# nka77/DAHiTra

Hardware: NVIDIA B200
Metric: image-pairs/sec (higher is better)
Workload: dtype x3 error-compensated f16 products (f16 main + scaled-remainder corrections; decoder: 3xTF32), fp32 accumulate

## Files before the change

dahitra_b200/csrc/stem_tc.cu:

```cuda
#include "tc_common.cuh"

using namespace dhtc;

namespace {
constexpr int SK_TH = 8, SK_TW = 16;
constexpr int SK_HR = 2 * SK_TH + 5;
constexpr int SK_HCP = 40;
constexpr int SK_PLANE = SK_HR * SK_HCP;
constexpr int SK_KSTEPS = 6;
constexpr int SK_GROUPS = 21;
constexpr uint32_t SK_A_BYTES = 128 * 128;
constexpr uint32_t SK_B_BYTES = SK_KSTEPS * 64 * 128;
constexpr uint32_t SK_HALO_BYTES = 3 * SK_PLANE * 4;
constexpr uint32_t SK_HALO_STRIDE = 10112;
constexpr uint32_t SK_IDESC = umma_idesc_tf32(128, 64);
constexpr int SK_THREADS = 14 * 32;

template <bool X3> struct SkCfg {
  static constexpr uint32_t NA = X3 ? 4 : 2;
  static constexpr uint32_t NB = X3 ? 2 : 1;
  static constexpr uint32_t OFF_B = NA * SK_A_BYTES;
  static constexpr uint32_t OFF_H = OFF_B + NB * SK_B_BYTES;
  static constexpr uint32_t OFF_E = OFF_H + 2 * SK_HALO_STRIDE;
  static constexpr uint32_t SMEM = OFF_E + 4 * 4096 + 1024;
};

__device__ __forceinline__ float sk_tf32(float v) { return tf32_round(v); }

struct SkTile { int n, oy0, ox0; };
__device__ __forceinline__ SkTile sk_tile(int t, int tilesX, int tilesY) {
  SkTile r;
  r.ox0 = (t % tilesX) * SK_TW; t /= tilesX;
  r.oy0 = (t % tilesY) * SK_TH;
  r.n = t / tilesY;
  return r;
}

__device__ __forceinline__ void sk_halo_producer(const CUtensorMap* tmX, uint32_t halo_addr, uint64_t* halo_full, uint64_t* halo_free,
                                                 int tilesX, int tilesY, int ntiles, const CUtensorMap* tmX2 = nullptr, int nfirst = 1 << 30) {
  int it = 0;
  for (int tile = blockIdx.x; tile < ntiles; tile += gridDim.x, ++it) {
    const int hb = it & 1;
    if (it >= 2) mbar_wait(smem_u32(&halo_free[hb]), (uint32_t)(((it >> 1) - 1) & 1));
    const SkTile tl = sk_tile(tile, tilesX, tilesY);
    const uint32_t bar = smem_u32(&halo_full[hb]);
    mbar_expect_tx(bar, SK_HALO_BYTES);
    const bool second = tl.n >= nfirst;
    tma_load_4d(halo_addr + (uint32_t)hb * SK_HALO_STRIDE, second ? tmX2 : tmX, bar, 2 * tl.ox0 - 4, 2 * tl.oy0 - 3, 0, second ? tl.n - nfirst : tl.n);
  }
}

__device__ __forceinline__ void sk_store_slice(const float (&v)[32], float* stage, int lane, int q, int j, const SkTile& t,
                                               int OH, int OW, const float* __restrict__ bias, float* __restrict__ out,
                                               long long split_plane = 0) {
  const int c4 = lane & 3, r4 = lane >> 2;
#pragma unroll
  for (int k4 = 0; k4 < 8; ++k4)
    *reinterpret_cast<float4*>(stage + lane * 32 + ((k4 ^ (lane & 7)) << 2)) = make_float4(v[k4 * 4], v[k4 * 4 + 1], v[k4 * 4 + 2], v[k4 * 4 + 3]);
  __syncwarp();
  const float4 b0 = ldg4(bias + j * 32 + c4 * 8), b1 = ldg4(bias + j * 32 + c4 * 8 + 4);
#pragma unroll
  for (int g = 0; g < 4; ++g) {
    const int r = g * 8 + r4, mm = q * 32 + r;
    const int oy = t.oy0 + mm / SK_TW, ox = t.ox0 + mm % SK_TW;
    const float4 o0 = *reinterpret_cast<const float4*>(stage + r * 32 + (((2 * c4) ^ (r & 7)) << 2));
    const float4 o1 = *reinterpret_cast<const float4*>(stage + r * 32 + (((2 * c4 + 1) ^ (r & 7)) << 2));
    if (oy < OH && ox < OW) {
      const float4 r0 = make_float4(fmaxf(o0.x + b0.x, 0.f), fmaxf(o0.y + b0.y, 0.f), fmaxf(o0.z + b0.z, 0.f), fmaxf(o0.w + b0.w, 0.f));
      const float4 r1 = make_float4(fmaxf(o1.x + b1.x, 0.f), fmaxf(o1.y + b1.y, 0.f), fmaxf(o1.z + b1.z, 0.f), fmaxf(o1.w + b1.w, 0.f));
      const size_t off = ((size_t)(t.n * OH + oy) * OW + ox) * 64 + j * 32 + c4 * 8;
      if (split_plane < 0) {
        uint4 hi;
        hi.x = pack_f16x2_sat(r0.x, r0.y); hi.y = pack_f16x2_sat(r0.z, r0.w); hi.z = pack_f16x2_sat(r1.x, r1.y); hi.w = pack_f16x2_sat(r1.z, r1.w);
        *reinterpret_cast<uint4*>(reinterpret_cast<uint16_t*>(out) + off) = hi;
      } else if (split_plane) {
        uint4 hi, lo;
        hi.x = pack_f16x2_sat(r0.x, r0.y); hi.y = pack_f16x2_sat(r0.z, r0.w); hi.z = pack_f16x2_sat(r1.x, r1.y); hi.w = pack_f16x2_sat(r1.z, r1.w);
        lo.x = pack_f16x2_sat((r0.x - f16_lo(hi.x)) * 2048.f, (r0.y - f16_hi(hi.x)) * 2048.f);
        lo.y = pack_f16x2_sat((r0.z - f16_lo(hi.y)) * 2048.f, (r0.w - f16_hi(hi.y)) * 2048.f);
        lo.z = pack_f16x2_sat((r1.x - f16_lo(hi.z)) * 2048.f, (r1.y - f16_hi(hi.z)) * 2048.f);
        lo.w = pack_f16x2_sat((r1.z - f16_lo(hi.w)) * 2048.f, (r1.w - f16_hi(hi.w)) * 2048.f);
        uint16_t* o16 = reinterpret_cast<uint16_t*>(out);
        *reinterpret_cast<uint4*>(o16 + off) = hi;
        *reinterpret_cast<uint4*>(o16 + off + (size_t)split_plane) = lo;
      } else {
        st4(out + off, r0); st4(out + off + 4, r1);
      }
    }
  }
  __syncwarp();
}

template <bool X3>
__global__ void __launch_bounds__(SK_THREADS, 1)
stem_tc_kernel(const __grid_constant__ CUtensorMap tmX, int OH, int OW, int tilesX, int tilesY, int ntiles,
               const float* __restrict__ wtc, const float* __restrict__ bias, float* __restrict__ out) {
  using Cfg = SkCfg<X3>;
  extern __shared__ uint8_t sk_raw[];
  __shared__ __align__(8) uint64_t w_bar, a_full[2], a_free[2], acc_full[2], acc_empty[2], halo_full[2], halo_free[2];
  __shared__ uint32_t tmem_slot;
  const int tid = threadIdx.x, warp = tid >> 5;
  const uint32_t base = (smem_u32(sk_raw) + 1023u) & ~1023u;
  uint8_t* bp = sk_raw + (base - smem_u32(sk_raw));
  constexpr uint32_t A_LO = 2 * SK_A_BYTES;
  const uint32_t b_addr = base + Cfg::OFF_B;

  if (tid == 0) {
    mbar_init(smem_u32(&w_bar), 1);
    for (int i = 0; i < 2; ++i) {
      mbar_init(smem_u32(&a_full[i]), 128);
      mbar_init(smem_u32(&a_free[i]), 1);
      mbar_init(smem_u32(&acc_full[i]), 1);
      mbar_init(smem_u32(&acc_empty[i]), 128);
      mbar_init(smem_u32(&halo_full[i]), 1);
      mbar_init(smem_u32(&halo_free[i]), 256);
    }
    mbar_fence_init();
  }
  if (warp == 0) tmem_alloc(smem_u32(&tmem_slot), 128);
  tc_fence_before();
  __syncthreads();
  tc_fence_after();
  const uint32_t tmem_base = tmem_slot;

  if (warp < 8) {
    const int wg = warp >> 2, t = tid & 127;
    const int py = t / SK_TW, px = t % SK_TW;
    const int pbase = (2 * py) * SK_HCP + 2 * px;
    const int swz = t & 7;
    int it = 0, use = 0;
    for (int tile = blockIdx.x; tile < ntiles; tile += gridDim.x, ++it) {
      const int hb = it & 1;
      mbar_wait(smem_u32(&halo_full[hb]), (uint32_t)((it >> 1) & 1));
      const float* halo = reinterpret_cast<const float*>(bp + Cfg::OFF_H + (size_t)hb * SK_HALO_STRIDE) + pbase;
      float* at = reinterpret_cast<float*>(bp + (size_t)wg * SK_A_BYTES) + t * 32;
#pragma unroll 1
      for (int kt = wg; kt < SK_KSTEPS; kt += 2, ++use) {
        if (use >= 1) mbar_wait(smem_u32(&a_free[wg]), (uint32_t)((use - 1) & 1));
#pragma unroll
        for (int j = 0; j < 4; ++j) {
          const int g = kt * 4 + j;
          float v[8];
          if (g < SK_GROUPS) {
            const float2* src = reinterpret_cast<const float2*>(halo + (g / 7) * SK_PLANE + (g % 7) * SK_HCP);
#pragma unroll
            for (int q = 0; q < 4; ++q) { const float2 f = src[q]; v[2 * q] = f.x; v[2 * q + 1] = f.y; }
          } else {
#pragma unroll
            for (int q = 0; q < 8; ++q) v[q] = 0.f;
          }
#pragma unroll
          for (int c = 0; c < 2; ++c) {
            const int o = ((2 * j + c) ^ swz) << 2;
            const float h0 = sk_tf32(v[c * 4]), h1 = sk_tf32(v[c * 4 + 1]), h2 = sk_tf32(v[c * 4 + 2]), h3 = sk_tf32(v[c * 4 + 3]);
            *reinterpret_cast<float4*>(at + o) = make_float4(h0, h1, h2, h3);
            if (X3) *reinterpret_cast<float4*>(at + A_LO / 4 + o) = make_float4(sk_tf32(v[c * 4] - h0), sk_tf32(v[c * 4 + 1] - h1),
                                                                              sk_tf32(v[c * 4 + 2] - h2), sk_tf32(v[c * 4 + 3] - h3));
          }
        }
        fence_async_smem();
        mbar_arrive_local(smem_u32(&a_full[wg]));
      }
      mbar_arrive_local(smem_u32(&halo_free[hb]));
    }
  } else if (warp < 12) {
    const int q = warp & 3, lane = tid & 31;
    float* stage = reinterpret_cast<float*>(bp + Cfg::OFF_E + (size_t)q * 4096);
    int it = 0;
    for (int tile = blockIdx.x; tile < ntiles; tile += gridDim.x, ++it) {
      const SkTile t = sk_tile(tile, tilesX, tilesY);
      const int ab = it & 1;
      mbar_wait(smem_u32(&acc_full[ab]), (uint32_t)((it >> 1) & 1));
      tc_fence_after();
      const uint32_t tm = tmem_base + ((uint32_t)(q * 32) << 16) + (uint32_t)ab * 64;
#pragma unroll 1
      for (int j = 0; j < 2; ++j) {
        uint32_t u[32];
        float v[32];
        tmem_ld32(tm + (uint32_t)(j * 32), u);
        if (j == 1) {
          tc_fence_before();
          mbar_arrive_local(smem_u32(&acc_empty[ab]));
        }
#pragma unroll
        for (int i = 0; i < 32; ++i) v[i] = __uint_as_float(u[i]);
        sk_store_slice(v, stage, lane, q, j, t, OH, OW, bias, out);
      }
    }
  } else if (warp == 13) {
    if ((tid & 31) == 0) sk_halo_producer(&tmX, base + Cfg::OFF_H, halo_full, halo_free, tilesX, tilesY, ntiles);
  } else if ((tid & 31) == 0) {
    mbar_expect_tx(smem_u32(&w_bar), Cfg::NB * SK_B_BYTES);
    bulk_load_1d(b_addr, wtc, SK_B_BYTES, smem_u32(&w_bar));
    if (X3) bulk_load_1d(b_addr + SK_B_BYTES, wtc + SK_B_BYTES / 4, SK_B_BYTES, smem_u32(&w_bar));
    mbar_wait(smem_u32(&w_bar), 0);
    int it = 0;
    uint32_t full_phase[2] = {0, 0};
    for (int tile = blockIdx.x; tile < ntiles; tile += gridDim.x, ++it) {
      const int ab = it & 1;
      mbar_wait(smem_u32(&acc_empty[ab]), (uint32_t)(((it >> 1) & 1) ^ 1));
      tc_fence_after();
      const uint32_t d = tmem_base + (uint32_t)ab * 64;
#pragma unroll
      for (int kt = 0; kt < SK_KSTEPS; ++kt) {
        const int buf = kt & 1;
        mbar_wait(smem_u32(&a_full[buf]), full_phase[buf]);
        full_phase[buf] ^= 1u;
        tc_fence_after();
        const uint32_t a_addr = base + (uint32_t)buf * SK_A_BYTES;
        const uint64_t ad = umma_desc_sw128(a_addr), bd = umma_desc_sw128(b_addr + (uint32_t)kt * 64 * 128);
#pragma unroll
        for (int k = 0; k < 4; ++k) umma_tf32(d, ad + (uint64_t)(2 * k), bd + (uint64_t)(2 * k), SK_IDESC, (kt | k) ? 1u : 0u);
        if (X3) {
          const uint64_t al = umma_desc_sw128(a_addr + A_LO), bl = umma_desc_sw128(b_addr + SK_B_BYTES + (uint32_t)kt * 64 * 128);
#pragma unroll
          for (int k = 0; k < 4; ++k) umma_tf32(d, al + (uint64_t)(2 * k), bd + (uint64_t)(2 * k), SK_IDESC, 1u);
#pragma unroll
          for (int k = 0; k < 4; ++k) umma_tf32(d, ad + (uint64_t)(2 * k), bl + (uint64_t)(2 * k), SK_IDESC, 1u);
        }
        umma_commit(smem_u32(&a_free[buf]));
      }
      umma_commit(smem_u32(&acc_full[ab]));
    }
  }
  tc_fence_before();
  __syncthreads();
  if (warp == 0) {
    tc_fence_after();
    tmem_dealloc(tmem_base, 128);
  }
}
constexpr int SF_KSTEPS = 3;
constexpr int SF_NBUF = 3;
constexpr uint32_t SF_A_BUF = 2 * SK_A_BYTES;
constexpr uint32_t SF_BM_STEP = 128 * 128;
constexpr uint32_t SF_BC_STEP = 64 * 128;
constexpr uint32_t SF_BM_BYTES = SF_KSTEPS * SF_BM_STEP, SF_BC_BYTES = SF_KSTEPS * SF_BC_STEP;
constexpr uint32_t SF_OFF_B = SF_NBUF * SF_A_BUF;
constexpr uint32_t SF_OFF_H = SF_OFF_B + SF_BM_BYTES + SF_BC_BYTES;
constexpr uint32_t SF_OFF_E = SF_OFF_H + 2 * SK_HALO_STRIDE;
constexpr uint32_t SF_SMEM = SF_OFF_E + 4 * 4096 + 1024;
constexpr uint32_t SF_IDESC_MAIN = umma_idesc_f16(128, 128), SF_IDESC_CORR = umma_idesc_bf16(128, 64), SF_IDESC_ONE = umma_idesc_f16(128, 64);
constexpr size_t SF_IMAGE_OFFSET_FLOATS = 2 * (SK_B_BYTES / 4);

template <bool FOLD>
__global__ void __launch_bounds__(SK_THREADS, 1)
stem_f16_kernel(const __grid_constant__ CUtensorMap tmX, const __grid_constant__ CUtensorMap tmX2, int nfirst, int OH, int OW, int tilesX,
                int tilesY, int ntiles, const float* __restrict__ wtc, const float* __restrict__ bias, float* __restrict__ out,
                long long split_plane) {
  extern __shared__ uint8_t sk_raw[];
  __shared__ __align__(8) uint64_t w_bar, a_full[SF_NBUF], a_free[SF_NBUF], acc_full[2], acc_empty[2], halo_full[2], halo_free[2];
  __shared__ uint32_t tmem_slot;
  const int tid = threadIdx.x, warp = tid >> 5;
  const uint32_t base = (smem_u32(sk_raw) + 1023u) & ~1023u;
  uint8_t* bp = sk_raw + (base - smem_u32(sk_raw));
  const uint32_t b_addr = base + SF_OFF_B;

  if (tid == 0) {
    mbar_init(smem_u32(&w_bar), 1);
    for (int i = 0; i < SF_NBUF; ++i) {
      mbar_init(smem_u32(&a_full[i]), 128);
      mbar_init(smem_u32(&a_free[i]), 1);
    }
    for (int i = 0; i < 2; ++i) {
      mbar_init(smem_u32(&acc_full[i]), 1);
      mbar_init(smem_u32(&acc_empty[i]), 128);
      mbar_init(smem_u32(&halo_full[i]), 1);
      mbar_init(smem_u32(&halo_free[i]), 256);
    }
    mbar_fence_init();
  }
  if (warp == 0) tmem_alloc(smem_u32(&tmem_slot), 256);
  tc_fence_before();
  __syncthreads();
  tc_fence_after();
  const uint32_t tmem_base = tmem_slot;
  dh_pdl_wait();
  dh_pdl_launch_dependents();

  if (warp < 8) {
    const int wg = warp >> 2, t = tid & 127;
    const int py = t / SK_TW, px = t % SK_TW;
    const int pbase = (2 * py) * SK_HCP + 2 * px;
    const int swz = t & 7;
    int it = 0, c = wg, buf = wg, use = 0;
    for (int tile = blockIdx.x; tile < ntiles; tile += gridDim.x, ++it) {
      const int hb = it & 1;
      mbar_wait(smem_u32(&halo_full[hb]), (uint32_t)((it >> 1) & 1));
      const float* halo = reinterpret_cast<const float*>(bp + SF_OFF_H + (size_t)hb * SK_HALO_STRIDE) + pbase;
#pragma unroll 1
      for (; c < SF_KSTEPS * (it + 1); c += 2) {
        const int kt = c - SF_KSTEPS * it;
        if (use >= 1) mbar_wait(smem_u32(&a_free[buf]), (uint32_t)((use - 1) & 1));
        uint8_t* row = bp + (size_t)buf * SF_A_BUF + t * 128;
        const int ng = kt == 2 ? 6 : 8;
#pragma unroll
        for (int j = 0; j < 8; ++j) {
          if (j < ng) {
            const int g = kt * 8 + j;
            uint4 hi = make_uint4(0u, 0u, 0u, 0u), lo = hi;
            if (g < SK_GROUPS) {
              const float2* src = reinterpret_cast<const float2*>(halo + (g / 7) * SK_PLANE + (g % 7) * SK_HCP);
              const float2 f0 = src[0], f1 = src[1], f2 = src[2], f3 = src[3];
              hi.x = pack_f16x2_sat(f0.x, f0.y); hi.y = pack_f16x2_sat(f1.x, f1.y);
              hi.z = pack_f16x2_sat(f2.x, f2.y); hi.w = pack_f16x2_sat(f3.x, f3.y);
              lo.x = pack_bf16x2(f0.x - f16_lo(hi.x), f0.y - f16_hi(hi.x)); lo.y = pack_bf16x2(f1.x - f16_lo(hi.y), f1.y - f16_hi(hi.y));
              lo.z = pack_bf16x2(f2.x - f16_lo(hi.z), f2.y - f16_hi(hi.z)); lo.w = pack_bf16x2(f3.x - f16_lo(hi.w), f3.y - f16_hi(hi.w));
            }
            const int o = (j ^ swz) << 4;
            *reinterpret_cast<uint4*>(row + o) = hi;
            if (FOLD) *reinterpret_cast<uint4*>(row + SK_A_BYTES + o) = lo;
          }
        }
        fence_async_smem();
        mbar_arrive_local(smem_u32(&a_full[buf]));
        buf += 2;
        if (buf >= SF_NBUF) { buf -= SF_NBUF; ++use; }
      }
      mbar_arrive_local(smem_u32(&halo_free[hb]));
    }
  } else if (warp < 12) {
    const int q = warp & 3, lane = tid & 31;
    float* stage = reinterpret_cast<float*>(bp + SF_OFF_E + (size_t)q * 4096);
    int it = 0;
    for (int tile = blockIdx.x; tile < ntiles; tile += gridDim.x, ++it) {
      const SkTile t = sk_tile(tile, tilesX, tilesY);
      const int ab = it & 1;
      mbar_wait(smem_u32(&acc_full[ab]), (uint32_t)((it >> 1) & 1));
      tc_fence_after();
      const uint32_t tm = tmem_base + ((uint32_t)(q * 32) << 16) + (uint32_t)ab * 128;
#pragma unroll 1
      for (int j = 0; j < 2; ++j) {
        uint32_t u[32], r[32];
        float v[32];
        tmem_ld32(tm + (uint32_t)(j * 32), u);
        if (FOLD) tmem_ld32(tm + (uint32_t)(64 + j * 32), r);
        if (j == 1) {
          tc_fence_before();
          mbar_arrive_local(smem_u32(&acc_empty[ab]));
        }
#pragma unroll
        for (int i = 0; i < 32; ++i) v[i] = FOLD ? fmaf(__uint_as_float(r[i]), 0x1p-11f, __uint_as_float(u[i])) : __uint_as_float(u[i]);
        sk_store_slice(v, stage, lane, q, j, t, OH, OW, bias, out, split_plane);
      }
    }
  } else if (warp == 13) {
    if ((tid & 31) == 0) sk_halo_producer(&tmX, base + SF_OFF_H, halo_full, halo_free, tilesX, tilesY, ntiles, &tmX2, nfirst);
  } else if ((tid & 31) == 0) {
    mbar_expect_tx(smem_u32(&w_bar), SF_BM_BYTES + SF_BC_BYTES);
    bulk_load_1d(b_addr, wtc + SF_IMAGE_OFFSET_FLOATS, SF_BM_BYTES, smem_u32(&w_bar));
    bulk_load_1d(b_addr + SF_BM_BYTES, wtc + SF_IMAGE_OFFSET_FLOATS + SF_BM_BYTES / 4, SF_BC_BYTES, smem_u32(&w_bar));
    mbar_wait(smem_u32(&w_bar), 0);
    int it = 0, buf = 0;
    uint32_t ph = 0;
    for (int tile = blockIdx.x; tile < ntiles; tile += gridDim.x, ++it) {
      const int ab = it & 1;
      mbar_wait(smem_u32(&acc_empty[ab]), (uint32_t)(((it >> 1) & 1) ^ 1));
      tc_fence_after();
      const uint32_t d = tmem_base + (uint32_t)ab * 128;
#pragma unroll
      for (int kt = 0; kt < SF_KSTEPS; ++kt) {
        mbar_wait(smem_u32(&a_full[buf]), ph);
        tc_fence_after();
        const uint32_t a_addr = base + (uint32_t)buf * SF_A_BUF;
        const uint64_t ah = umma_desc_sw128(a_addr), al = umma_desc_sw128(a_addr + SK_A_BYTES);
        const uint64_t bm = umma_desc_sw128(b_addr + (uint32_t)kt * SF_BM_STEP);
        const uint64_t bc = umma_desc_sw128(b_addr + SF_BM_BYTES + (uint32_t)kt * SF_BC_STEP);
        constexpr int NK = 4;
#pragma unroll
        for (int k = 0; k < NK; ++k)
          if (kt < 2 || k < 3) umma_bf16(d, ah + (uint64_t)(2 * k), bm + (uint64_t)(2 * k), FOLD ? SF_IDESC_MAIN : SF_IDESC_ONE, (kt | k) ? 1u : 0u);
        if (FOLD) {
#pragma unroll
          for (int k = 0; k < NK; ++k)
            if (kt < 2 || k < 3) umma_bf16(d, al + (uint64_t)(2 * k), bc + (uint64_t)(2 * k), SF_IDESC_CORR, 1u);
        }
        umma_commit(smem_u32(&a_free[buf]));
        if (++buf == SF_NBUF) { buf = 0; ph ^= 1u; }
      }
      umma_commit(smem_u32(&acc_full[ab]));
    }
  }
  tc_fence_before();
  __syncthreads();
  if (warp == 0) {
    tc_fence_after();
    tmem_dealloc(tmem_base, 256);
  }
}
}

int dh_launch_stem_tc(const float* x, long long xbs, int N, int H, int W, const float* wtc, const float* b, float* out,
                      int x3, cudaStream_t s, long long split_plane_pitch, const float* x_second) {
  const bool split = (x3 & 256) != 0, h16 = (x3 & 512) != 0;
  DH_REQUIRE(!(x3 & ~(255 | 256 | 512)) && !(split && h16), DH_E_VARIANT);
  x3 &= 255;
  DH_REQUIRE(!x_second || x3 == 2 || x3 == 3, DH_E_VARIANT);
  DH_REQUIRE(!split || x3 == 2 || x3 == 3, DH_E_VARIANT);
  DH_REQUIRE(!h16 || x3 == 3, DH_E_VARIANT);
  DH_REQUIRE(x && wtc && b && out, DH_E_NULL);
  DH_REQUIRE(N > 0 && H >= 8 && W >= 8 && H % 2 == 0 && W % 2 == 0, DH_E_SHAPE);
  DH_REQUIRE(dh_aligned16(wtc) && dh_aligned16(b) && dh_aligned16(out), DH_E_ALIGN);
  DH_REQUIRE((reinterpret_cast<uintptr_t>(x) & 3u) == 0, DH_E_ALIGN);
  const int OH = H / 2, OW = W / 2;
  const int tx = dh_cdiv(OW, SK_TW), ty = dh_cdiv(OH, SK_TH);
  const int nimg = x_second ? 2 * N : N;
  const int ntiles = tx * ty * nimg;
  const long long split_plane = h16 ? -1 : split ? (split_plane_pitch ? split_plane_pitch : (long long)nimg * OH * OW * 64) : 0;
  int dev = 0, sms = 148;
  cudaGetDevice(&dev);
  cudaDeviceGetAttribute(&sms, cudaDevAttrMultiProcessorCount, dev);
  dim3 grid((unsigned)(ntiles < sms ? ntiles : sms), 1, 1);
  DH_REQUIRE(W % 4 == 0 && xbs % 4 == 0 && dh_aligned16(x), DH_E_ALIGN);
  CUtensorMap tmX;
  {
    const unsigned long long dims[4] = {(unsigned long long)W, (unsigned long long)H, 3ull, (unsigned long long)N};
    const unsigned long long strides[3] = {(unsigned long long)W * 4, (unsigned long long)H * W * 4, (unsigned long long)xbs * 4};
    const unsigned box[4] = {(unsigned)SK_HCP, (unsigned)SK_HR, 3u, 1u};
    const int rc = dh_encode_tiled_f32(&tmX, x, 4, dims, strides, box, false);
    if (rc) return rc;
  }
  CUtensorMap tmX2 = tmX;
  if (x_second) {
    DH_REQUIRE(dh_aligned16(x_second), DH_E_ALIGN);
    const unsigned long long dims[4] = {(unsigned long long)W, (unsigned long long)H, 3ull, (unsigned long long)N};
    const unsigned long long strides[3] = {(unsigned long long)W * 4, (unsigned long long)H * W * 4, (unsigned long long)xbs * 4};
    const unsigned box[4] = {(unsigned)SK_HCP, (unsigned)SK_HR, 3u, 1u};
    const int rc = dh_encode_tiled_f32(&tmX2, x_second, 4, dims, strides, box, false);
    if (rc) return rc;
  }
  const int nfirst = x_second ? N : (1 << 30);
  if (x3 == 2) {
    cudaError_t e = cudaFuncSetAttribute(stem_f16_kernel<true>, cudaFuncAttributeMaxDynamicSharedMemorySize, (int)SF_SMEM);
    if (e != cudaSuccess) return (int)e;
    return dh_launch(stem_f16_kernel<true>, grid, dim3(SK_THREADS), SF_SMEM, s, tmX, tmX2, nfirst, OH, OW, tx, ty, ntiles, wtc, b, out, split_plane);
  } else if (x3 == 3) {
    cudaError_t e = cudaFuncSetAttribute(stem_f16_kernel<false>, cudaFuncAttributeMaxDynamicSharedMemorySize, (int)SF_SMEM);
    if (e != cudaSuccess) return (int)e;
    return dh_launch(stem_f16_kernel<false>, grid, dim3(SK_THREADS), SF_SMEM, s, tmX, tmX2, nfirst, OH, OW, tx, ty, ntiles, wtc, b, out, split_plane);
  } else if (x3) {
    cudaError_t e = cudaFuncSetAttribute(stem_tc_kernel<true>, cudaFuncAttributeMaxDynamicSharedMemorySize, (int)SkCfg<true>::SMEM);
    if (e != cudaSuccess) return (int)e;
    stem_tc_kernel<true><<<grid, SK_THREADS, SkCfg<true>::SMEM, s>>>(tmX, OH, OW, tx, ty, ntiles, wtc, b, out);
  } else {
    cudaError_t e = cudaFuncSetAttribute(stem_tc_kernel<false>, cudaFuncAttributeMaxDynamicSharedMemorySize, (int)SkCfg<false>::SMEM);
    if (e != cudaSuccess) return (int)e;
    stem_tc_kernel<false><<<grid, SK_THREADS, SkCfg<false>::SMEM, s>>>(tmX, OH, OW, tx, ty, ntiles, wtc, b, out);
  }
  DH_CHECK_LAUNCH();
  return 0;
}
```

dahitra_b200/csrc/tc_common.cuh:

```cuda
#pragma once
#include "common.cuh"
#include <cuda.h>
#include <cstdio>

int dh_encode_tiled_f32(CUtensorMap* out, const void* ptr, int rank, const unsigned long long* dims,
                        const unsigned long long* strides, const unsigned* box, bool swizzle128);
int dh_encode_tiled_f32_sw(CUtensorMap* out, const void* ptr, int rank, const unsigned long long* dims,
                           const unsigned long long* strides, const unsigned* box, int swizzle_bytes);
int dh_encode_tiled_f16_sw(CUtensorMap* out, const void* ptr, int rank, const unsigned long long* dims,
                           const unsigned long long* strides, const unsigned* box, int swizzle_bytes);

namespace dhtc {

__device__ __forceinline__ uint32_t smem_u32(const void* p) { return (uint32_t)__cvta_generic_to_shared(p); }

__device__ __forceinline__ void mbar_init(uint32_t bar, uint32_t count) {
  asm volatile("mbarrier.init.shared::cta.b64 [%0], %1;" ::"r"(bar), "r"(count) : "memory");
}
__device__ __forceinline__ void mbar_fence_init() { asm volatile("fence.mbarrier_init.release.cluster;" ::: "memory"); }
__device__ __forceinline__ void mbar_expect_tx(uint32_t bar, uint32_t bytes) {
  asm volatile("mbarrier.arrive.expect_tx.shared::cta.b64 _, [%0], %1;" ::"r"(bar), "r"(bytes) : "memory");
}
__device__ __forceinline__ void pdl_wait() { asm volatile("griddepcontrol.wait;" ::: "memory"); }
__device__ __forceinline__ void pdl_launch_dependents() { asm volatile("griddepcontrol.launch_dependents;" ::: "memory"); }

__device__ __forceinline__ void mbar_wait(uint32_t bar, uint32_t parity) {
  uint32_t done;
#ifdef DH_MBAR_TIMEOUT
  uint32_t spins = 0;
#endif
  do {
    asm volatile(
        "{\n\t.reg .pred p;\n\t"
        "mbarrier.try_wait.parity.shared::cta.b64 p, [%1], %2, %3;\n\t"
        "selp.u32 %0, 1, 0, p;\n\t}"
        : "=r"(done) : "r"(bar), "r"(parity), "r"(10000u) : "memory");
#ifdef DH_MBAR_TIMEOUT
    if (!done && ++spins > (1u << 19)) {
      printf("[mbar timeout] block %d thread %d bar smem+0x%x parity %u\n", blockIdx.x, threadIdx.x, bar, parity);
      __trap();
    }
#endif
  } while (!done);
}
__device__ __forceinline__ uint32_t cluster_ctarank() { uint32_t r; asm volatile("mov.u32 %0, %%cluster_ctarank;" : "=r"(r)); return r; }
__device__ __forceinline__ void cluster_sync_all() {
  asm volatile("barrier.cluster.arrive.release.aligned;" ::: "memory");
  asm volatile("barrier.cluster.wait.acquire.aligned;" ::: "memory");
}
__device__ __forceinline__ uint32_t mapa_u32(uint32_t smem_addr, uint32_t rank) {
  uint32_t r;
  asm volatile("mapa.shared::cluster.u32 %0, %1, %2;" : "=r"(r) : "r"(smem_addr), "r"(rank));
  return r;
}
__device__ __forceinline__ void mbar_arrive_local(uint32_t bar) {
  asm volatile("mbarrier.arrive.shared::cta.b64 _, [%0];" ::"r"(bar) : "memory");
}
__device__ __forceinline__ void mbar_arrive_cluster(uint32_t cluster_bar) {
  asm volatile("mbarrier.arrive.release.cluster.shared::cluster.b64 _, [%0];" ::"r"(cluster_bar) : "memory");
}
__device__ __forceinline__ void mbar_wait_cluster(uint32_t bar, uint32_t parity) {
  uint32_t done;
#ifdef DH_MBAR_TIMEOUT
  uint32_t spins = 0;
#endif
  do {
    asm volatile(
        "{\n\t.reg .pred p;\n\t"
        "mbarrier.try_wait.parity.acquire.cluster.shared::cta.b64 p, [%1], %2, %3;\n\t"
        "selp.u32 %0, 1, 0, p;\n\t}"
        : "=r"(done) : "r"(bar), "r"(parity), "r"(10000u) : "memory");
#ifdef DH_MBAR_TIMEOUT
    if (!done && ++spins > (1u << 19)) __trap();
#endif
  } while (!done);
}
__device__ __forceinline__ void tma_load_4d_2sm(uint32_t dst, const CUtensorMap* tm, uint32_t cluster_bar, int c0, int c1, int c2, int c3) {
  asm volatile(
      "cp.async.bulk.tensor.4d.cta_group::2.shared::cluster.global.tile.mbarrier::complete_tx::bytes [%0], [%1, {%3, %4, %5, %6}], [%2];"
      ::"r"(dst), "l"(tm), "r"(cluster_bar), "r"(c0), "r"(c1), "r"(c2), "r"(c3) : "memory");
}
__device__ __forceinline__ void tma_load_2d_2sm(uint32_t dst, const CUtensorMap* tm, uint32_t cluster_bar, int c0, int c1) {
  asm volatile(
      "cp.async.bulk.tensor.2d.cta_group::2.shared::cluster.global.tile.mbarrier::complete_tx::bytes [%0], [%1, {%3, %4}], [%2];"
      ::"r"(dst), "l"(tm), "r"(cluster_bar), "r"(c0), "r"(c1) : "memory");
}
__device__ __forceinline__ float tf32_round(float v) {
  return __uint_as_float((__float_as_uint(v) + 0x1000u) & 0xFFFFE000u);
}
__device__ __forceinline__ void tma_load_4d(uint32_t dst, const CUtensorMap* tm, uint32_t bar, int c0, int c1, int c2, int c3) {
  asm volatile(
      "cp.async.bulk.tensor.4d.shared::cluster.global.tile.mbarrier::complete_tx::bytes [%0], [%1, {%3, %4, %5, %6}], [%2];"
      ::"r"(dst), "l"(tm), "r"(bar), "r"(c0), "r"(c1), "r"(c2), "r"(c3) : "memory");
}
__device__ __forceinline__ void tma_load_2d(uint32_t dst, const CUtensorMap* tm, uint32_t bar, int c0, int c1) {
  asm volatile(
      "cp.async.bulk.tensor.2d.shared::cluster.global.tile.mbarrier::complete_tx::bytes [%0], [%1, {%3, %4}], [%2];"
      ::"r"(dst), "l"(tm), "r"(bar), "r"(c0), "r"(c1) : "memory");
}
__device__ __forceinline__ void bulk_load_1d(uint32_t dst, const void* src, uint32_t bytes, uint32_t bar) {
  asm volatile("cp.async.bulk.shared::cluster.global.mbarrier::complete_tx::bytes [%0], [%1], %2, [%3];"
               ::"r"(dst), "l"(src), "r"(bytes), "r"(bar) : "memory");
}
__device__ __forceinline__ void fence_async_smem() { asm volatile("fence.proxy.async.shared::cta;" ::: "memory"); }
__device__ __forceinline__ void tc_fence_before() { asm volatile("tcgen05.fence::before_thread_sync;" ::: "memory"); }
__device__ __forceinline__ void tc_fence_after() { asm volatile("tcgen05.fence::after_thread_sync;" ::: "memory"); }

__device__ __forceinline__ uint64_t umma_desc_sw128(uint32_t smem_addr) {
  return (uint64_t)((smem_addr & 0x3FFFF) >> 4) | ((uint64_t)1 << 16) | ((uint64_t)(1024 >> 4) << 32) |
         ((uint64_t)1 << 46) | ((uint64_t)2 << 61);
}
__host__ __device__ constexpr uint32_t umma_idesc_tf32(int M, int N) {
  return (1u << 4) | (2u << 7) | (2u << 10) | ((uint32_t)(N >> 3) << 17) | ((uint32_t)(M >> 4) << 24);
}
__device__ __forceinline__ void umma_tf32(uint32_t tmem_d, uint64_t adesc, uint64_t bdesc, uint32_t idesc, uint32_t accumulate) {
  asm volatile(
      "{\n\t.reg .pred p;\n\t"
      "setp.ne.b32 p, %4, 0;\n\t"
      "tcgen05.mma.cta_group::1.kind::tf32 [%0], %1, %2, %3, p;\n\t}"
      ::"r"(tmem_d), "l"(adesc), "l"(bdesc), "r"(idesc), "r"(accumulate) : "memory");
}
__device__ __forceinline__ uint64_t umma_desc_sw64(uint32_t smem_addr, uint32_t sbo_bytes) {
  return (uint64_t)((smem_addr & 0x3FFFF) >> 4) | ((uint64_t)1 << 16) | ((uint64_t)(sbo_bytes >> 4) << 32) |
         ((uint64_t)1 << 46) | ((uint64_t)4 << 61);
}
__host__ __device__ constexpr uint32_t umma_idesc_bf16(int M, int N) {
  return (1u << 4) | (1u << 7) | (1u << 10) | ((uint32_t)(N >> 3) << 17) | ((uint32_t)(M >> 4) << 24);
}
__device__ __forceinline__ void umma_bf16(uint32_t tmem_d, uint64_t adesc, uint64_t bdesc, uint32_t idesc, uint32_t accumulate) {
  asm volatile(
      "{\n\t.reg .pred p;\n\t"
      "setp.ne.b32 p, %4, 0;\n\t"
      "tcgen05.mma.cta_group::1.kind::f16 [%0], %1, %2, %3, p;\n\t}"
      ::"r"(tmem_d), "l"(adesc), "l"(bdesc), "r"(idesc), "r"(accumulate) : "memory");
}
__host__ __device__ constexpr uint32_t umma_idesc_f16(int M, int N) {
  return (1u << 4) | ((uint32_t)(N >> 3) << 17) | ((uint32_t)(M >> 4) << 24);
}
__device__ __forceinline__ uint32_t pack_f16x2_sat(float lo, float hi) {
  uint32_t r;
  asm("cvt.rn.satfinite.f16x2.f32 %0, %1, %2;" : "=r"(r) : "f"(hi), "f"(lo));
  return r;
}
__device__ __forceinline__ float f16_lo(uint32_t p) { float f; asm("{ .reg .b16 l, h; mov.b32 {l, h}, %1; cvt.f32.f16 %0, l; }" : "=f"(f) : "r"(p)); return f; }
__device__ __forceinline__ float f16_hi(uint32_t p) { float f; asm("{ .reg .b16 l, h; mov.b32 {l, h}, %1; cvt.f32.f16 %0, h; }" : "=f"(f) : "r"(p)); return f; }
__device__ __forceinline__ uint32_t pack_bf16x2(float lo, float hi) {
  uint32_t r;
  asm("cvt.rn.bf16x2.f32 %0, %1, %2;" : "=r"(r) : "f"(hi), "f"(lo));
  return r;
}
__device__ __forceinline__ void umma_tf32_ts(uint32_t tmem_d, uint32_t tmem_a, uint64_t bdesc, uint32_t idesc, uint32_t accumulate) {
  asm volatile(
      "{\n\t.reg .pred p;\n\t"
      "setp.ne.b32 p, %4, 0;\n\t"
      "tcgen05.mma.cta_group::1.kind::tf32 [%0], [%1], %2, %3, p;\n\t}"
      ::"r"(tmem_d), "r"(tmem_a), "l"(bdesc), "r"(idesc), "r"(accumulate) : "memory");
}
__device__ __forceinline__ void umma_tf32_2sm(uint32_t tmem_d, uint64_t adesc, uint64_t bdesc, uint32_t idesc, uint32_t accumulate) {
  asm volatile(
      "{\n\t.reg .pred p;\n\t"
      "setp.ne.b32 p, %4, 0;\n\t"
      "tcgen05.mma.cta_group::2.kind::tf32 [%0], %1, %2, %3, p;\n\t}"
      ::"r"(tmem_d), "l"(adesc), "l"(bdesc), "r"(idesc), "r"(accumulate) : "memory");
}
__device__ __forceinline__ void umma_bf16_2sm(uint32_t tmem_d, uint64_t adesc, uint64_t bdesc, uint32_t idesc, uint32_t accumulate) {
  asm volatile(
      "{\n\t.reg .pred p;\n\t"
      "setp.ne.b32 p, %4, 0;\n\t"
      "tcgen05.mma.cta_group::2.kind::f16 [%0], %1, %2, %3, p;\n\t}"
      ::"r"(tmem_d), "l"(adesc), "l"(bdesc), "r"(idesc), "r"(accumulate) : "memory");
}
__device__ __forceinline__ void umma_commit_2sm(uint32_t bar) {
  asm volatile("tcgen05.commit.cta_group::2.mbarrier::arrive::one.shared::cluster.multicast::cluster.b64 [%0], %1;"
               ::"r"(bar), "h"((uint16_t)3) : "memory");
}
__device__ __forceinline__ void tmem_alloc_2sm(uint32_t slot_smem_addr, uint32_t ncols) {
  asm volatile("tcgen05.alloc.cta_group::2.sync.aligned.shared::cta.b32 [%0], %1;" ::"r"(slot_smem_addr), "r"(ncols) : "memory");
  asm volatile("tcgen05.relinquish_alloc_permit.cta_group::2.sync.aligned;" ::: "memory");
}
__device__ __forceinline__ void tmem_dealloc_2sm(uint32_t taddr, uint32_t ncols) {
  asm volatile("tcgen05.dealloc.cta_group::2.sync.aligned.b32 %0, %1;" ::"r"(taddr), "r"(ncols) : "memory");
}
__device__ __forceinline__ void umma_commit(uint32_t bar) {
  asm volatile("tcgen05.commit.cta_group::1.mbarrier::arrive::one.shared::cluster.b64 [%0];" ::"r"(bar) : "memory");
}
__device__ __forceinline__ void tmem_alloc(uint32_t slot_smem_addr, uint32_t ncols) {
  asm volatile("tcgen05.alloc.cta_group::1.sync.aligned.shared::cta.b32 [%0], %1;" ::"r"(slot_smem_addr), "r"(ncols) : "memory");
  asm volatile("tcgen05.relinquish_alloc_permit.cta_group::1.sync.aligned;" ::: "memory");
}
__device__ __forceinline__ void tmem_dealloc(uint32_t taddr, uint32_t ncols) {
  asm volatile("tcgen05.dealloc.cta_group::1.sync.aligned.b32 %0, %1;" ::"r"(taddr), "r"(ncols) : "memory");
}
__device__ __forceinline__ void tmem_ld32(uint32_t taddr, uint32_t (&v)[32]) {
  asm volatile(
      "tcgen05.ld.sync.aligned.32x32b.x32.b32 "
      "{%0, %1, %2, %3, %4, %5, %6, %7, %8, %9, %10, %11, %12, %13, %14, %15, "
      "%16, %17, %18, %19, %20, %21, %22, %23, %24, %25, %26, %27, %28, %29, %30, %31}, [%32];"
      : "=r"(v[0]), "=r"(v[1]), "=r"(v[2]), "=r"(v[3]), "=r"(v[4]), "=r"(v[5]), "=r"(v[6]), "=r"(v[7]),
        "=r"(v[8]), "=r"(v[9]), "=r"(v[10]), "=r"(v[11]), "=r"(v[12]), "=r"(v[13]), "=r"(v[14]), "=r"(v[15]),
        "=r"(v[16]), "=r"(v[17]), "=r"(v[18]), "=r"(v[19]), "=r"(v[20]), "=r"(v[21]), "=r"(v[22]), "=r"(v[23]),
        "=r"(v[24]), "=r"(v[25]), "=r"(v[26]), "=r"(v[27]), "=r"(v[28]), "=r"(v[29]), "=r"(v[30]), "=r"(v[31])
      : "r"(taddr) : "memory");
  asm volatile("tcgen05.wait::ld.sync.aligned;" ::: "memory");
}
__device__ __forceinline__ void tmem_ld16(uint32_t taddr, uint32_t (&v)[16]) {
  asm volatile(
      "tcgen05.ld.sync.aligned.32x32b.x16.b32 "
      "{%0, %1, %2, %3, %4, %5, %6, %7, %8, %9, %10, %11, %12, %13, %14, %15}, [%16];"
      : "=r"(v[0]), "=r"(v[1]), "=r"(v[2]), "=r"(v[3]), "=r"(v[4]), "=r"(v[5]), "=r"(v[6]), "=r"(v[7]),
        "=r"(v[8]), "=r"(v[9]), "=r"(v[10]), "=r"(v[11]), "=r"(v[12]), "=r"(v[13]), "=r"(v[14]), "=r"(v[15])
      : "r"(taddr) : "memory");
  asm volatile("tcgen05.wait::ld.sync.aligned;" ::: "memory");
}
__device__ __forceinline__ void tmem_st32(uint32_t taddr, const uint32_t (&v)[32]) {
  asm volatile(
      "tcgen05.st.sync.aligned.32x32b.x32.b32 [%0], "
      "{%1, %2, %3, %4, %5, %6, %7, %8, %9, %10, %11, %12, %13, %14, %15, %16, "
      "%17, %18, %19, %20, %21, %22, %23, %24, %25, %26, %27, %28, %29, %30, %31, %32};"
      ::"r"(taddr), "r"(v[0]), "r"(v[1]), "r"(v[2]), "r"(v[3]), "r"(v[4]), "r"(v[5]), "r"(v[6]), "r"(v[7]),
        "r"(v[8]), "r"(v[9]), "r"(v[10]), "r"(v[11]), "r"(v[12]), "r"(v[13]), "r"(v[14]), "r"(v[15]),
        "r"(v[16]), "r"(v[17]), "r"(v[18]), "r"(v[19]), "r"(v[20]), "r"(v[21]), "r"(v[22]), "r"(v[23]),
        "r"(v[24]), "r"(v[25]), "r"(v[26]), "r"(v[27]), "r"(v[28]), "r"(v[29]), "r"(v[30]), "r"(v[31])
      : "memory");
  asm volatile("tcgen05.wait::st.sync.aligned;" ::: "memory");
}

__device__ __forceinline__ unsigned long long f2_pack(float2 a) { unsigned long long r; asm("mov.b64 %0, {%1, %2};" : "=l"(r) : "f"(a.x), "f"(a.y)); return r; }
__device__ __forceinline__ float2 f2_unpack(unsigned long long r) { float2 d; asm("mov.b64 {%0, %1}, %2;" : "=f"(d.x), "=f"(d.y) : "l"(r)); return d; }
__device__ __forceinline__ float2 ffma2(float2 a, float2 b, float2 c) {
  unsigned long long d; asm("fma.rn.f32x2 %0, %1, %2, %3;" : "=l"(d) : "l"(f2_pack(a)), "l"(f2_pack(b)), "l"(f2_pack(c))); return f2_unpack(d);
}
__device__ __forceinline__ float2 fadd2(float2 a, float2 b) { unsigned long long d; asm("add.rn.f32x2 %0, %1, %2;" : "=l"(d) : "l"(f2_pack(a)), "l"(f2_pack(b))); return f2_unpack(d); }
__device__ __forceinline__ float2 fsub2(float2 a, float2 b) { unsigned long long d; asm("sub.rn.f32x2 %0, %1, %2;" : "=l"(d) : "l"(f2_pack(a)), "l"(f2_pack(b))); return f2_unpack(d); }
__device__ __forceinline__ float2 fmul2(float2 a, float2 b) { unsigned long long d; asm("mul.rn.f32x2 %0, %1, %2;" : "=l"(d) : "l"(f2_pack(a)), "l"(f2_pack(b))); return f2_unpack(d); }
__device__ __forceinline__ float2 f2_bcast(float s) { return make_float2(s, s); }

__host__ __device__ __forceinline__ int sw128_idx(int r, int k) { return r * 32 + ((((k >> 2) ^ (r & 7)) << 2) | (k & 3)); }

}
```

Baseline: 17260.

## Stage stem A operands in tensor memory instead of shared memory for f16 MMA

The stem f16 kernel now writes the hi/lo split A operands straight into tensor memory with tcgen05.st and issues MMAs that take A from TMEM. Shared-memory A buffers are dropped, and the ring grows to four buffers inside a 512-column TMEM allocation. The goal is to cut shared-memory store traffic and bandwidth contention on the MMA A path. The cost is a full 512-column TMEM allocation, extra tcgen05 fences and waits on the producer side, and the risk that the TMEM A layout does not match what the MMA expects. The old shared-memory path stays available behind a flag bit.

Result: no change. 17410 (median of 6 runs) (+0.8%).

```diff
diff --git a/dahitra_b200/csrc/stem_tc.cu b/dahitra_b200/csrc/stem_tc.cu
--- a/dahitra_b200/csrc/stem_tc.cu
+++ b/dahitra_b200/csrc/stem_tc.cu
@@ -233,32 +233,52 @@
 constexpr int SF_KSTEPS = 3;
 constexpr int SF_NBUF = 3;
 constexpr uint32_t SF_A_BUF = 2 * SK_A_BYTES;
+constexpr uint32_t SF_TM_A = 256, SF_TM_A_BUF = 64;
 constexpr uint32_t SF_BM_STEP = 128 * 128;
 constexpr uint32_t SF_BC_STEP = 64 * 128;
 constexpr uint32_t SF_BM_BYTES = SF_KSTEPS * SF_BM_STEP, SF_BC_BYTES = SF_KSTEPS * SF_BC_STEP;
-constexpr uint32_t SF_OFF_B = SF_NBUF * SF_A_BUF;
-constexpr uint32_t SF_OFF_H = SF_OFF_B + SF_BM_BYTES + SF_BC_BYTES;
-constexpr uint32_t SF_OFF_E = SF_OFF_H + 2 * SK_HALO_STRIDE;
-constexpr uint32_t SF_SMEM = SF_OFF_E + 4 * 4096 + 1024;
+template <bool A_TMEM> struct SfCfg {
+  static constexpr int NBUF = A_TMEM ? 4 : SF_NBUF;
+  static constexpr uint32_t OFF_B = A_TMEM ? 0 : SF_NBUF * SF_A_BUF;
+  static constexpr uint32_t OFF_H = OFF_B + SF_BM_BYTES + SF_BC_BYTES;
+  static constexpr uint32_t OFF_E = OFF_H + 2 * SK_HALO_STRIDE;
+  static constexpr uint32_t SMEM = OFF_E + 4 * 4096 + 1024;
+  static constexpr uint32_t TMEM_COLS = A_TMEM ? 512 : 256;
+};
 constexpr uint32_t SF_IDESC_MAIN = umma_idesc_f16(128, 128), SF_IDESC_CORR = umma_idesc_bf16(128, 64), SF_IDESC_ONE = umma_idesc_f16(128, 64);
 constexpr size_t SF_IMAGE_OFFSET_FLOATS = 2 * (SK_B_BYTES / 4);
 
-template <bool FOLD>
+__device__ __forceinline__ void sf_group(const float* halo, int g, uint4& hi, uint4& lo) {
+  hi = make_uint4(0u, 0u, 0u, 0u);
+  lo = hi;
+  if (g < SK_GROUPS) {
+    const float2* src = reinterpret_cast<const float2*>(halo + (g / 7) * SK_PLANE + (g % 7) * SK_HCP);
+    const float2 f0 = src[0], f1 = src[1], f2 = src[2], f3 = src[3];
+    hi.x = pack_f16x2_sat(f0.x, f0.y); hi.y = pack_f16x2_sat(f1.x, f1.y);
+    hi.z = pack_f16x2_sat(f2.x, f2.y); hi.w = pack_f16x2_sat(f3.x, f3.y);
+    lo.x = pack_bf16x2(f0.x - f16_lo(hi.x), f0.y - f16_hi(hi.x)); lo.y = pack_bf16x2(f1.x - f16_lo(hi.y), f1.y - f16_hi(hi.y));
+    lo.z = pack_bf16x2(f2.x - f16_lo(hi.z), f2.y - f16_hi(hi.z)); lo.w = pack_bf16x2(f3.x - f16_lo(hi.w), f3.y - f16_hi(hi.w));
+  }
+}
+
+template <bool FOLD, bool A_TMEM>
 __global__ void __launch_bounds__(SK_THREADS, 1)
 stem_f16_kernel(const __grid_constant__ CUtensorMap tmX, const __grid_constant__ CUtensorMap tmX2, int nfirst, int OH, int OW, int tilesX,
                 int tilesY, int ntiles, const float* __restrict__ wtc, const float* __restrict__ bias, float* __restrict__ out,
                 long long split_plane) {
+  using Cfg = SfCfg<A_TMEM>;
   extern __shared__ uint8_t sk_raw[];
-  __shared__ __align__(8) uint64_t w_bar, a_full[SF_NBUF], a_free[SF_NBUF], acc_full[2], acc_empty[2], halo_full[2], halo_free[2];
+  constexpr int NBUF = Cfg::NBUF;
+  __shared__ __align__(8) uint64_t w_bar, a_full[NBUF], a_free[NBUF], acc_full[2], acc_empty[2], halo_full[2], halo_free[2];
   __shared__ uint32_t tmem_slot;
   const int tid = threadIdx.x, warp = tid >> 5;
   const uint32_t base = (smem_u32(sk_raw) + 1023u) & ~1023u;
   uint8_t* bp = sk_raw + (base - smem_u32(sk_raw));
-  const uint32_t b_addr = base + SF_OFF_B;
+  const uint32_t b_addr = base + Cfg::OFF_B;
 
   if (tid == 0) {
     mbar_init(smem_u32(&w_bar), 1);
-    for (int i = 0; i < SF_NBUF; ++i) {
+    for (int i = 0; i < NBUF; ++i) {
       mbar_init(smem_u32(&a_full[i]), 128);
       mbar_init(smem_u32(&a_free[i]), 1);
     }
@@ -270,7 +290,7 @@
     }
     mbar_fence_init();
   }
-  if (warp == 0) tmem_alloc(smem_u32(&tmem_slot), 256);
+  if (warp == 0) tmem_alloc(smem_u32(&tmem_slot), Cfg::TMEM_COLS);
   tc_fence_before();
   __syncthreads();
   tc_fence_after();
@@ -283,45 +303,60 @@
     const int py = t / SK_TW, px = t % SK_TW;
     const int pbase = (2 * py) * SK_HCP + 2 * px;
     const int swz = t & 7;
+    const uint32_t a_lane = tmem_base + ((uint32_t)((warp & 3) * 32) << 16) + SF_TM_A;
     int it = 0, c = wg, buf = wg, use = 0;
     for (int tile = blockIdx.x; tile < ntiles; tile += gridDim.x, ++it) {
       const int hb = it & 1;
       mbar_wait(smem_u32(&halo_full[hb]), (uint32_t)((it >> 1) & 1));
-      const float* halo = reinterpret_cast<const float*>(bp + SF_OFF_H + (size_t)hb * SK_HALO_STRIDE) + pbase;
+      const float* halo = reinterpret_cast<const float*>(bp + Cfg::OFF_H + (size_t)hb * SK_HALO_STRIDE) + pbase;
 #pragma unroll 1
       for (; c < SF_KSTEPS * (it + 1); c += 2) {
         const int kt = c - SF_KSTEPS * it;
-        if (use >= 1) mbar_wait(smem_u32(&a_free[buf]), (uint32_t)((use - 1) & 1));
-        uint8_t* row = bp + (size_t)buf * SF_A_BUF + t * 128;
-        const int ng = kt == 2 ? 6 : 8;
-#pragma unroll
-        for (int j = 0; j < 8; ++j) {
-          if (j < ng) {
-            const int g = kt * 8 + j;
-            uint4 hi = make_uint4(0u, 0u, 0u, 0u), lo = hi;
-            if (g < SK_GROUPS) {
-              const float2* src = reinterpret_cast<const float2*>(halo + (g / 7) * SK_PLANE + (g % 7) * SK_HCP);
-              const float2 f0 = src[0], f1 = src[1], f2 = src[2], f3 = src[3];
-              hi.x = pack_f16x2_sat(f0.x, f0.y); hi.y = pack_f16x2_sat(f1.x, f1.y);
-              hi.z = pack_f16x2_sat(f2.x, f2.y); hi.w = pack_f16x2_sat(f3.x, f3.y);
-              lo.x = pack_bf16x2(f0.x - f16_lo(hi.x), f0.y - f16_hi(hi.x)); lo.y = pack_bf16x2(f1.x - f16_lo(hi.y), f1.y - f16_hi(hi.y));
-              lo.z = pack_bf16x2(f2.x - f16_lo(hi.z), f2.y - f16_hi(hi.z)); lo.w = pack_bf16x2(f3.x - f16_lo(hi.w), f3.y - f16_hi(hi.w));
+        if (use >= 1) {
+          mbar_wait(smem_u32(&a_free[buf]), (uint32_t)((use - 1) & 1));
+          if (A_TMEM) tc_fence_after();
+        }
+        if constexpr (A_TMEM) {
+          const uint32_t arow = a_lane + (uint32_t)buf * SF_TM_A_BUF;
+#pragma unroll
+          for (int h = 0; h < 2; ++h) {
+            uint32_t hi[16], lo[16];
+#pragma unroll
+            for (int j = 0; j < 4; ++j) {
+              uint4 gh, gl;
+              sf_group(halo, kt * 8 + h * 4 + j, gh, gl);
+              hi[4 * j] = gh.x; hi[4 * j + 1] = gh.y; hi[4 * j + 2] = gh.z; hi[4 * j + 3] = gh.w;
+              lo[4 * j] = gl.x; lo[4 * j + 1] = gl.y; lo[4 * j + 2] = gl.z; lo[4 * j + 3] = gl.w;
             }
-            const int o = (j ^ swz) << 4;
-            *reinterpret_cast<uint4*>(row + o) = hi;
-            if (FOLD) *reinterpret_cast<uint4*>(row + SK_A_BYTES + o) = lo;
+            tmem_st16_nowait(arow + (uint32_t)(16 * h), hi);
+            if (FOLD) tmem_st16_nowait(arow + 32u + (uint32_t)(16 * h), lo);
           }
-        }
-        fence_async_smem();
+          tmem_wait_st();
+          tc_fence_before();
+        } else {
+          uint8_t* row = bp + (size_t)buf * SF_A_BUF + t * 128;
+          const int ng = kt == 2 ? 6 : 8;
+#pragma unroll
+          for (int j = 0; j < 8; ++j) {
+            if (j < ng) {
+              uint4 hi, lo;
+              sf_group(halo, kt * 8 + j, hi, lo);
+              const int o = (j ^ swz) << 4;
+              *reinterpret_cast<uint4*>(row + o) = hi;
+              if (FOLD) *reinterpret_cast<uint4*>(row + SK_A_BYTES + o) = lo;
+            }
+          }
+          fence_async_smem();
+        }
         mbar_arrive_local(smem_u32(&a_full[buf]));
         buf += 2;
-        if (buf >= SF_NBUF) { buf -= SF_NBUF; ++use; }
+        if (buf >= NBUF) { buf -= NBUF; ++use; }
       }
       mbar_arrive_local(smem_u32(&halo_free[hb]));
     }
   } else if (warp < 12) {
     const int q = warp & 3, lane = tid & 31;
-    float* stage = reinterpret_cast<float*>(bp + SF_OFF_E + (size_t)q * 4096);
+    float* stage = reinterpret_cast<float*>(bp + Cfg::OFF_E + (size_t)q * 4096);
     int it = 0;
     for (int tile = blockIdx.x; tile < ntiles; tile += gridDim.x, ++it) {
       const SkTile t = sk_tile(tile, tilesX, tilesY);
@@ -345,7 +380,7 @@
       }
     }
   } else if (warp == 13) {
-    if ((tid & 31) == 0) sk_halo_producer(&tmX, base + SF_OFF_H, halo_full, halo_free, tilesX, tilesY, ntiles, &tmX2, nfirst);
+    if ((tid & 31) == 0) sk_halo_producer(&tmX, base + Cfg::OFF_H, halo_full, halo_free, tilesX, tilesY, ntiles, &tmX2, nfirst);
   } else if ((tid & 31) == 0) {
     mbar_expect_tx(smem_u32(&w_bar), SF_BM_BYTES + SF_BC_BYTES);
     bulk_load_1d(b_addr, wtc + SF_IMAGE_OFFSET_FLOATS, SF_BM_BYTES, smem_u32(&w_bar));
@@ -362,21 +397,33 @@
       for (int kt = 0; kt < SF_KSTEPS; ++kt) {
         mbar_wait(smem_u32(&a_full[buf]), ph);
         tc_fence_after();
-        const uint32_t a_addr = base + (uint32_t)buf * SF_A_BUF;
-        const uint64_t ah = umma_desc_sw128(a_addr), al = umma_desc_sw128(a_addr + SK_A_BYTES);
         const uint64_t bm = umma_desc_sw128(b_addr + (uint32_t)kt * SF_BM_STEP);
         const uint64_t bc = umma_desc_sw128(b_addr + SF_BM_BYTES + (uint32_t)kt * SF_BC_STEP);
         constexpr int NK = 4;
-#pragma unroll
-        for (int k = 0; k < NK; ++k)
-          if (kt < 2 || k < 3) umma_bf16(d, ah + (uint64_t)(2 * k), bm + (uint64_t)(2 * k), FOLD ? SF_IDESC_MAIN : SF_IDESC_ONE, (kt | k) ? 1u : 0u);
-        if (FOLD) {
+        if constexpr (A_TMEM) {
+          const uint32_t ah = tmem_base + SF_TM_A + (uint32_t)buf * SF_TM_A_BUF, al = ah + 32u;
 #pragma unroll
           for (int k = 0; k < NK; ++k)
-            if (kt < 2 || k < 3) umma_bf16(d, al + (uint64_t)(2 * k), bc + (uint64_t)(2 * k), SF_IDESC_CORR, 1u);
+            if (kt < 2 || k < 3) umma_bf16_ts(d, ah + 8u * k, bm + (uint64_t)(2 * k), FOLD ? SF_IDESC_MAIN : SF_IDESC_ONE, (kt | k) ? 1u : 0u);
+          if (FOLD) {
+#pragma unroll
+            for (int k = 0; k < NK; ++k)
+              if (kt < 2 || k < 3) umma_bf16_ts(d, al + 8u * k, bc + (uint64_t)(2 * k), SF_IDESC_CORR, 1u);
+          }
+        } else {
+          const uint32_t a_addr = base + (uint32_t)buf * SF_A_BUF;
+          const uint64_t ah = umma_desc_sw128(a_addr), al = umma_desc_sw128(a_addr + SK_A_BYTES);
+#pragma unroll
+          for (int k = 0; k < NK; ++k)
+            if (kt < 2 || k < 3) umma_bf16(d, ah + (uint64_t)(2 * k), bm + (uint64_t)(2 * k), FOLD ? SF_IDESC_MAIN : SF_IDESC_ONE, (kt | k) ? 1u : 0u);
+          if (FOLD) {
+#pragma unroll
+            for (int k = 0; k < NK; ++k)
+              if (kt < 2 || k < 3) umma_bf16(d, al + (uint64_t)(2 * k), bc + (uint64_t)(2 * k), SF_IDESC_CORR, 1u);
+          }
         }
         umma_commit(smem_u32(&a_free[buf]));
-        if (++buf == SF_NBUF) { buf = 0; ph ^= 1u; }
+        if (++buf == NBUF) { buf = 0; ph ^= 1u; }
       }
       umma_commit(smem_u32(&acc_full[ab]));
     }
@@ -385,18 +432,28 @@
   __syncthreads();
   if (warp == 0) {
     tc_fence_after();
-    tmem_dealloc(tmem_base, 256);
-  }
+    tmem_dealloc(tmem_base, Cfg::TMEM_COLS);
+  }
+}
+
+template <bool FOLD, bool A_TMEM>
+int sf_launch(dim3 grid, cudaStream_t s, const CUtensorMap& tmX, const CUtensorMap& tmX2, int nfirst, int OH, int OW, int tx, int ty,
+              int ntiles, const float* wtc, const float* b, float* out, long long split_plane) {
+  constexpr uint32_t smem = SfCfg<A_TMEM>::SMEM;
+  cudaError_t e = cudaFuncSetAttribute(stem_f16_kernel<FOLD, A_TMEM>, cudaFuncAttributeMaxDynamicSharedMemorySize, (int)smem);
+  if (e != cudaSuccess) return (int)e;
+  return dh_launch(stem_f16_kernel<FOLD, A_TMEM>, grid, dim3(SK_THREADS), smem, s, tmX, tmX2, nfirst, OH, OW, tx, ty, ntiles, wtc, b, out, split_plane);
 }
 }
 
 int dh_launch_stem_tc(const float* x, long long xbs, int N, int H, int W, const float* wtc, const float* b, float* out,
                       int x3, cudaStream_t s, long long split_plane_pitch, const float* x_second) {
-  const bool split = (x3 & 256) != 0, h16 = (x3 & 512) != 0;
-  DH_REQUIRE(!(x3 & ~(255 | 256 | 512)) && !(split && h16), DH_E_VARIANT);
+  const bool split = (x3 & 256) != 0, h16 = (x3 & 512) != 0, smem_a = (x3 & 1024) != 0;
+  DH_REQUIRE(!(x3 & ~(255 | 256 | 512 | 1024)) && !(split && h16), DH_E_VARIANT);
   x3 &= 255;
   DH_REQUIRE(!x_second || x3 == 2 || x3 == 3, DH_E_VARIANT);
   DH_REQUIRE(!split || x3 == 2 || x3 == 3, DH_E_VARIANT);
+  DH_REQUIRE(!smem_a || x3 == 2 || x3 == 3, DH_E_VARIANT);
   DH_REQUIRE(!h16 || x3 == 3, DH_E_VARIANT);
   DH_REQUIRE(x && wtc && b && out, DH_E_NULL);
   DH_REQUIRE(N > 0 && H >= 8 && W >= 8 && H % 2 == 0 && W % 2 == 0, DH_E_SHAPE);
@@ -430,14 +487,10 @@
     if (rc) return rc;
   }
   const int nfirst = x_second ? N : (1 << 30);
-  if (x3 == 2) {
-    cudaError_t e = cudaFuncSetAttribute(stem_f16_kernel<true>, cudaFuncAttributeMaxDynamicSharedMemorySize, (int)SF_SMEM);
-    if (e != cudaSuccess) return (int)e;
-    return dh_launch(stem_f16_kernel<true>, grid, dim3(SK_THREADS), SF_SMEM, s, tmX, tmX2, nfirst, OH, OW, tx, ty, ntiles, wtc, b, out, split_plane);
-  } else if (x3 == 3) {
-    cudaError_t e = cudaFuncSetAttribute(stem_f16_kernel<false>, cudaFuncAttributeMaxDynamicSharedMemorySize, (int)SF_SMEM);
-    if (e != cudaSuccess) return (int)e;
-    return dh_launch(stem_f16_kernel<false>, grid, dim3(SK_THREADS), SF_SMEM, s, tmX, tmX2, nfirst, OH, OW, tx, ty, ntiles, wtc, b, out, split_plane);
+  if (x3 == 2 || x3 == 3) {
+    auto launch = x3 == 2 ? (smem_a ? sf_launch<true, false> : sf_launch<true, true>)
+                          : (smem_a ? sf_launch<false, false> : sf_launch<false, true>);
+    return launch(grid, s, tmX, tmX2, nfirst, OH, OW, tx, ty, ntiles, wtc, b, out, split_plane);
   } else if (x3) {
     cudaError_t e = cudaFuncSetAttribute(stem_tc_kernel<true>, cudaFuncAttributeMaxDynamicSharedMemorySize, (int)SkCfg<true>::SMEM);
     if (e != cudaSuccess) return (int)e;
diff --git a/dahitra_b200/csrc/tc_common.cuh b/dahitra_b200/csrc/tc_common.cuh
--- a/dahitra_b200/csrc/tc_common.cuh
+++ b/dahitra_b200/csrc/tc_common.cuh
@@ -154,6 +154,13 @@
       "{\n\t.reg .pred p;\n\t"
       "setp.ne.b32 p, %4, 0;\n\t"
       "tcgen05.mma.cta_group::1.kind::tf32 [%0], [%1], %2, %3, p;\n\t}"
+      ::"r"(tmem_d), "r"(tmem_a), "l"(bdesc), "r"(idesc), "r"(accumulate) : "memory");
+}
+__device__ __forceinline__ void umma_bf16_ts(uint32_t tmem_d, uint32_t tmem_a, uint64_t bdesc, uint32_t idesc, uint32_t accumulate) {
+  asm volatile(
+      "{\n\t.reg .pred p;\n\t"
+      "setp.ne.b32 p, %4, 0;\n\t"
+      "tcgen05.mma.cta_group::1.kind::f16 [%0], [%1], %2, %3, p;\n\t}"
       ::"r"(tmem_d), "r"(tmem_a), "l"(bdesc), "r"(idesc), "r"(accumulate) : "memory");
 }
 __device__ __forceinline__ void umma_tf32_2sm(uint32_t tmem_d, uint64_t adesc, uint64_t bdesc, uint32_t idesc, uint32_t accumulate) {
@@ -224,6 +231,15 @@
       : "memory");
   asm volatile("tcgen05.wait::st.sync.aligned;" ::: "memory");
 }
+__device__ __forceinline__ void tmem_st16_nowait(uint32_t taddr, const uint32_t (&v)[16]) {
+  asm volatile(
+      "tcgen05.st.sync.aligned.32x32b.x16.b32 [%0], "
+      "{%1, %2, %3, %4, %5, %6, %7, %8, %9, %10, %11, %12, %13, %14, %15, %16};"
+      ::"r"(taddr), "r"(v[0]), "r"(v[1]), "r"(v[2]), "r"(v[3]), "r"(v[4]), "r"(v[5]), "r"(v[6]), "r"(v[7]),
+        "r"(v[8]), "r"(v[9]), "r"(v[10]), "r"(v[11]), "r"(v[12]), "r"(v[13]), "r"(v[14]), "r"(v[15])
+      : "memory");
+}
+__device__ __forceinline__ void tmem_wait_st() { asm volatile("tcgen05.wait::st.sync.aligned;" ::: "memory"); }
 
 __device__ __forceinline__ unsigned long long f2_pack(float2 a) { unsigned long long r; asm("mov.b64 %0, {%1, %2};" : "=l"(r) : "f"(a.x), "f"(a.y)); return r; }
 __device__ __forceinline__ float2 f2_unpack(unsigned long long r) { float2 d; asm("mov.b64 {%0, %1}, %2;" : "=f"(d.x), "=f"(d.y) : "l"(r)); return d; }
```
